# url-kaist/patchwork-plusplus

Hardware: NVIDIA H100
Metric: frames/sec (120k-pt KITTI cloud) (higher is better)
Workload: dtype f64

## Files before the change

### patchwork-plusplus_b200/csrc/pwpp_capi.cu

```cuda
#include <cuda_runtime.h>

#include <sched.h>

#include <algorithm>
#include <cctype>
#include <chrono>
#include <cstdio>
#include <cstdlib>
#include <cstring>
#include <string>
#include <vector>

#include "pwpp.h"
#include "pwpp_kernels.cuh"
#include "pwpp_tuning.h"
#include "pwpp_host.hpp"

using namespace pwpp;

static_assert(sizeof(BinFit) == sizeof(pwpp_bin_result), "BinFit must mirror pwpp_bin_result");

namespace {

thread_local std::string g_last_error;
// ... 509 lines not shown
  pwpp_ctx* ctx = new pwpp_ctx();
  ctx->prm = *params;
  ctx->device = device;
  ctx->num_streams = num_streams;
  build_geometry(*params, ctx->g, ctx->ap, ctx->fast_bin);
  ctx->sw_serial_fit = env_int("PWPP_SERIAL_FIT", 0, 0, 1) != 0;
  ctx->sw_front = env_int("PWPP_FRONT", PWPP_FRONT_DEFAULT, 0, 1);
  ctx->sw_patch = env_int("PWPP_FIT_PATCH", PWPP_FIT_PATCH_DEFAULT, 0, 1);
  ctx->sw_graph = env_int("PWPP_GRAPH", 1, 0, 1);
  ctx->small_call_frames = env_int("PWPP_SMALL_CALL", PWPP_SMALL_CALL_DEFAULT, 0, 64);
  ctx->nbp = ((ctx->g.nbins + PW_NUM_PSEUDO + 31) / 32) * 32;
  int max_sectors = 0;
  for (int k = 0; k < 4; ++k) max_sectors = std::max(max_sectors, ctx->g.num_sectors[k]);
  ctx->hcap = std::max(params->max_elevation_storage, params->max_flatness_storage) + 4 * max_sectors + 64;
  ctx->max_sectors = max_sectors;
#define CU_TRY_CTX(expr)                                                                                  \
  do {                                                                                                    \
    cudaError_t _e = (expr);                                                                              \
    if (_e != cudaSuccess) {                                                                              \
      std::string m = std::string(#expr) + ": " + cudaGetErrorString(_e);                                 \
      pwpp_destroy(ctx);                                                                                  \
      return fail(PWPP_ERR_CUDA, m);                                                                      \
    }                                                                                                     \
  } while (0)
  CU_TRY_CTX(cudaSetDevice(device));
  CU_TRY_CTX(cudaStreamCreateWithFlags(&ctx->stream, cudaStreamNonBlocking));
  CU_TRY_CTX(cudaStreamCreateWithFlags(&ctx->stream_h2d, cudaStreamNonBlocking));
  CU_TRY_CTX(cudaStreamCreateWithFlags(&ctx->stream_d2h, cudaStreamNonBlocking));
  CU_TRY_CTX(cudaEventCreate(&ctx->ev0));
  CU_TRY_CTX(cudaEventCreate(&ctx->ev1));
  CU_TRY_CTX(cudaEventCreate(&ctx->ev_begin));
  CU_TRY_CTX(cudaEventCreate(&ctx->ev_end));
  for (int i = 0; i <= PWPP_NUM_STAGES; ++i) CU_TRY_CTX(cudaEventCreate(&ctx->stage_ev[i]));
  for (int i = 0; i < 2; ++i) CU_TRY_CTX(cudaEventCreateWithFlags(&ctx->tab_ev[i], cudaEventDisableTiming));
  CU_TRY_CTX(cudaEventCreateWithFlags(&ctx->ev_fork, cudaEventDisableTiming));
  for (int q = 0; q < NUM_SIDE; ++q) {
    CU_TRY_CTX(cudaStreamCreateWithFlags(&ctx->side[q], cudaStreamNonBlocking));
    CU_TRY_CTX(cudaEventCreateWithFlags(&ctx->ev_fit[q], cudaEventDisableTiming));
    CU_TRY_CTX(cudaEventCreateWithFlags(&ctx->ev_join[q], cudaEventDisableTiming));
  }
  CU_TRY_CTX(ctx->d_states.reserve(num_streams));
  CU_TRY_CTX(ctx->d_states_init.reserve(num_streams));
  {
    std::vector<StreamState> v(num_streams);
    for (auto& st : v) init_state(*params, st);
    CU_TRY_CTX(cudaMemcpy(ctx->d_states_init.p, v.data(), v.size() * sizeof(StreamState), cudaMemcpyHostToDevice));
  }
  CU_TRY_CTX(ctx->d_hist.reserve((size_t) num_streams * 2 * 4 * ctx->hcap));
  CU_TRY_CTX(ctx->d_counts.reserve((size_t) 3 * num_streams));
  CU_TRY_CTX(ctx->d_wq_ctr.reserve(2 * NUM_CLASSES + ORD_NUM_HEADS));
  {
    cudaDeviceProp prop;
    CU_TRY_CTX(cudaGetDeviceProperties(&prop, device));
    const size_t sm_m = FITW_WARPS * CLS_M_MAX * sizeof(float4), sm_l2 = 3 * 4096 * sizeof(float), sm_l3 = 3 * 8192 * sizeof(float);
    ctx->fit[0] = {k_fit_resident<8, 8, 0, 2>, 0, FIT_THREADS, 0};
    ctx->fit[1] = {k_fit_warp<true, 1, 1, 2, 3, false, true>, 0, FITW_WARPS * 32, sm_m};
    ctx->fit[2] = {k_fit_warp<false, 2, 2, 2, 3, false, true>, 0, FITW_WARPS * 32, 0};
    ctx->fit[3] = {k_fit_cta<4096, 3, 3, 8, true, true>, 0, FIT_THREADS, sm_l2};
    ctx->fit[4] = {k_fit_cta<8192, 4, 2, 8, true>, 0, FIT_THREADS, sm_l3};
    ctx->fit[5] = {k_fit_big<16, 1, true>, 0, 512, 0};
    if (ctx->sw_patch) {
      ctx->fit[2] = {k_fit_patch<4, 4, 2>, 0, 4 * 32, (size_t) 4 * FP_STG * sizeof(float4)};
      ctx->fit[3] = {k_fit_patch<8, 2, 3>, 0, 8 * 32, (size_t) 8 * FP_STG * sizeof(float4)};
      ctx->fit[4] = {k_fit_patch<16, 1, 4>, 0, 16 * 32, (size_t) 16 * FP_STG * sizeof(float4)};
    }
    for (int c = 0; c < NUM_CLASSES; ++c) ctx->fit_small[c] = ctx->fit[c];
    ctx->fit_small[2] = {k_fit_patch<4, 4, 2>, 0, 4 * 32, (size_t) 4 * FP_STG * sizeof(float4)};
    ctx->fit_small[3] = {k_fit_patch<8, 2, 3>, 0, 8 * 32, (size_t) 8 * FP_STG * sizeof(float4)};
    ctx->fit_small[4] = {k_fit_patch<16, 1, 4>, 0, 16 * 32, (size_t) 16 * FP_STG * sizeof(float4)};
    for (int c = 0; c < 2 * NUM_CLASSES; ++c) {
      FitLaunch& k = c < NUM_CLASSES ? ctx->fit[c] : ctx->fit_small[c - NUM_CLASSES];
      if (k.smem > 0) CU_TRY_CTX(cudaFuncSetAttribute(k.fn, cudaFuncAttributeMaxDynamicSharedMemorySize, (int) k.smem));
      int per_sm = 1;
      CU_TRY_CTX(cudaOccupancyMaxActiveBlocksPerMultiprocessor(&per_sm, k.fn, k.threads, k.smem));
      k.grid = std::max(1, per_sm) * prop.multiProcessorCount;
    }
    {
      typedef void (*OrdKernel)(const float4*, WorkQueues, int*, int*);
      const OrdKernel fn[ORD_NUM_HEADS] = {k_order_cta<512, 5>, k_order_cta<512, 4>, k_order_cta<256, 3>, k_order_cta<128, 2>, k_order_warp};
      const int th[ORD_NUM_HEADS] = {512, 512, 256, 128, ORD_WARP_THREADS};
      for (int q = 0; q < ORD_NUM_HEADS; ++q) {
        const size_t sm = q < 4 ? ord_cta_smem_bytes(th[q]) : 0;
        if (sm > 48 * 1024) CU_TRY_CTX(cudaFuncSetAttribute(fn[q], cudaFuncAttributeMaxDynamicSharedMemorySize, (int) sm));
        int per_sm = 1;
        CU_TRY_CTX(cudaOccupancyMaxActiveBlocksPerMultiprocessor(&per_sm, fn[q], th[q], sm));
        ctx->order_k[q].grid = std::max(1, per_sm) * prop.multiProcessorCount;
        ctx->order_k[q].threads = th[q];
        ctx->order_k[q].smem = sm;
      }
    }
    const size_t gle_smem = gle_smem_bytes(max_sectors);
    if (gle_smem > 48 * 1024) CU_TRY_CTX(cudaFuncSetAttribute(k_gle, cudaFuncAttributeMaxDynamicSharedMemorySize, (int) gle_smem));
  }
  {
    const size_t scat = (size_t) (CHUNK_THREADS / 32) * ctx->nbp * sizeof(unsigned int);
    if (scat > 48 * 1024) CU_TRY_CTX(cudaFuncSetAttribute(k_scatter<false, 4>, cudaFuncAttributeMaxDynamicSharedMemorySize, (int) scat));
    const size_t sm_f = front_cluster_smem_bytes(ctx->nbp, FC_THREADS), sm_fd = front_cluster_smem_bytes(ctx->nbp, FC_THREADS_DENSE);
    if (sm_f > 220 * 1024) ctx->sw_front = 0;
    ctx->front_dense_ok = sm_fd <= 220 * 1024;
    if (ctx->sw_front) {
      CU_TRY_CTX(cudaFuncSetAttribute(k_front_cluster<true, CLS_L2_MAX, FC_THREADS>, cudaFuncAttributeMaxDynamicSharedMemorySize, (int) sm_f));
      CU_TRY_CTX(cudaFuncSetAttribute(k_front_cluster<false, CLS_L2_MAX, FC_THREADS>, cudaFuncAttributeMaxDynamicSharedMemorySize, (int) sm_f));
      if (ctx->front_dense_ok) {
        CU_TRY_CTX(cudaFuncSetAttribute(k_front_cluster<true, CLS_L2_MAX, FC_THREADS_DENSE>, cudaFuncAttributeMaxDynamicSharedMemorySize, (int) sm_fd));
        CU_TRY_CTX(cudaFuncSetAttribute(k_front_cluster<false, CLS_L2_MAX, FC_THREADS_DENSE>, cudaFuncAttributeMaxDynamicSharedMemorySize, (int) sm_fd));
      }
    }
// ... 432 lines not shown
  int node = -1;
  if (FILE* f = std::fopen((base + "/numa_node").c_str(), "r")) { if (std::fscanf(f, "%d", &node) != 1) node = -1; std::fclose(f); }
  if (node < 0) return -1;
  std::string list;
  if (FILE* f = std::fopen(("/sys/devices/system/node/node" + std::to_string(node) + "/cpulist").c_str(), "r")) {
    char buf[4096] = {0};
    if (std::fgets(buf, sizeof buf, f)) list = buf;
    std::fclose(f);
  }
  if (list.empty()) return -1;
  cpu_set_t set;
  CPU_ZERO(&set);
  int ncpu = 0;
  const char* p = list.c_str();
  while (*p) {
    char* end = nullptr;
    long a = std::strtol(p, &end, 10);
    if (end == p) break;
    long b = a;
    if (*end == '-') { p = end + 1; b = std::strtol(p, &end, 10); }
    for (long c = a; c <= b && c < CPU_SETSIZE; ++c) { CPU_SET((int) c, &set); ++ncpu; }
    p = (*end == ',') ? end + 1 : end;
    if (*end != ',' ) break;
  }
  if (ncpu == 0 || sched_setaffinity(0, sizeof set, &set) != 0) return -1;
  return node;
}

int pwpp_copy_bin_results(pwpp_ctx* ctx, int f, pwpp_bin_result* dst) {
  int rc = check_frame(ctx, f);
  if (rc) return rc;
  rc = bind_device(ctx);
  if (rc) return rc;
  CU_TRY(cudaStreamSynchronize(ctx->last_stream));
  CU_TRY(cudaMemcpy(dst, ctx->d_fits.p + (size_t) f * ctx->g.nbins, (size_t) ctx->g.nbins * sizeof(BinFit), cudaMemcpyDeviceToHost));
  return PWPP_OK;
}
int pwpp_copy_bin_ids(pwpp_ctx* ctx, int f, uint16_t* dst) {
  int rc = check_frame(ctx, f);
  if (rc) return rc;
  rc = bind_device(ctx);
  if (rc) return rc;
  CU_TRY(cudaStreamSynchronize(ctx->last_stream));
  const int n = frame_n(ctx, f);
  if (n > 0) CU_TRY(cudaMemcpy(dst, ctx->d_bin_ids.p + ctx->pt_off[f], (size_t) n * sizeof(uint16_t), cudaMemcpyDeviceToHost));
  return PWPP_OK;
}

#if defined(PWPP_PHASE_CLOCKS)
int pwpp_debug_phase_clocks(pwpp_ctx* ctx, unsigned long long* out, int reset) {
  if (!ctx) return PWPP_ERR_INVALID_ARG;
  cudaSetDevice(ctx->device);
  cudaDeviceSynchronize();
  if (out) cudaMemcpyFromSymbol(out, g_phase_clk, sizeof(unsigned long long) * 48);
  if (reset) { static unsigned long long z[48]; cudaMemcpyToSymbol(g_phase_clk, z, sizeof z); }
  return PWPP_OK;
}
int pwpp_debug_events(pwpp_ctx* ctx, unsigned* out, int max_events) {
  if (!ctx) return -1;
  cudaSetDevice(ctx->device);
  cudaDeviceSynchronize();
  if (out && max_events >= 16384) cudaMemcpyFromSymbol(out, g_ev, (size_t) 16384 * 16);
  static uint4 z[16384];
  cudaMemcpyToSymbol(g_ev, z, sizeof z);
  return 16384;
}
#endif

}
```

### patchwork-plusplus_b200/csrc/pwpp_common.cuh

```cuda
#pragma once
#include <cuda_runtime.h>

#include "pwpp_gle.cuh"
#include "pwpp_math.cuh"

namespace pwpp {

constexpr int CHUNK_PTS = 4096;
constexpr int CHUNK_THREADS = 256;
constexpr int WARP_PTS = CHUNK_PTS / (CHUNK_THREADS / 32);
constexpr int WARP_ITERS = WARP_PTS / 32;
constexpr int MAX_LPR = 64;
constexpr int MAX_RVPF = 8;

struct FrameTable {
  const long long* pt_off;
  const int* chunk_off;
};

__device__ __forceinline__ int lane_id() { return threadIdx.x & 31; }
#if defined(PWPP_SIMT_EMU)
__device__ __forceinline__ unsigned pw_cluster_rank() { return blockIdx.x; }
__device__ __forceinline__ void pw_cluster_sync() { simt::cluster_sync_(); }
template <typename T> __device__ __forceinline__ T* pw_cluster_map(T* p, unsigned rank) { return static_cast<T*>(simt::cluster_map_(p, (int) rank)); }
#else
}
#include <cooperative_groups.h>
namespace pwpp {
__device__ __forceinline__ unsigned pw_cluster_rank() { return cooperative_groups::this_cluster().block_rank(); }
__device__ __forceinline__ void pw_cluster_sync() { cooperative_groups::this_cluster().sync(); }
template <typename T> __device__ __forceinline__ T* pw_cluster_map(T* p, unsigned rank) { return cooperative_groups::this_cluster().map_shared_rank(p, rank); }
#endif

#if defined(PWPP_SIMT_EMU)
__device__ __forceinline__ unsigned lanemask_lt() { return (1u << (threadIdx.x & 31)) - 1u; }
__device__ __forceinline__ float4 ld_stream_f4(const float4* p) { return *p; }
__device__ __forceinline__ void prefetch_l2(const void*) {}
#else
#define PW_DYN_SHARED(T, name) extern __shared__ T name[]
__device__ __forceinline__ unsigned lanemask_lt() { unsigned m; asm("mov.u32 %0, %%lanemask_lt;" : "=r"(m)); return m; }

__device__ __forceinline__ float4 ld_stream_f4(const float4* p) {
  float4 v;
  asm("ld.global.nc.L1::no_allocate.v4.f32 {%0,%1,%2,%3}, [%4];" : "=f"(v.x), "=f"(v.y), "=f"(v.z), "=f"(v.w) : "l"(p));
  return v;
}
__device__ __forceinline__ void prefetch_l2(const void* p) { asm volatile("prefetch.global.L2 [%0];" ::"l"(p)); }
#endif

#if !defined(PWPP_SIMT_EMU)
__device__ __forceinline__ unsigned smem_u32(const void* p) { return (unsigned) __cvta_generic_to_shared(p); }
__device__ __forceinline__ void mbar_init(unsigned long long* bar, int count) {
  asm volatile("mbarrier.init.shared::cta.b64 [%0], %1;" ::"r"(smem_u32(bar)), "r"(count) : "memory");
}
__device__ __forceinline__ void mbar_expect_tx(unsigned long long* bar, unsigned bytes) {
  asm volatile("mbarrier.arrive.expect_tx.shared::cta.b64 _, [%0], %1;" ::"r"(smem_u32(bar)), "r"(bytes) : "memory");
}
__device__ __forceinline__ void mbar_wait(unsigned long long* bar, unsigned parity) {
  asm volatile(
      "{\n"
      ".reg .pred p;\n"
      "WAIT_%=:\n"
      "mbarrier.try_wait.parity.shared::cta.b64 p, [%0], %1;\n"
      "@p bra DONE_%=;\n"
      "bra WAIT_%=;\n"
      "DONE_%=:\n"
      "}\n" ::"r"(smem_u32(bar)), "r"(parity) : "memory");
}
__device__ __forceinline__ void bulk_g2s(void* dst_smem, const void* src_gmem, unsigned bytes, unsigned long long* bar) {
  asm volatile("cp.async.bulk.shared::cta.global.mbarrier::complete_tx::bytes [%0], [%1], %2, [%3];" ::"r"(smem_u32(dst_smem)), "l"(src_gmem), "r"(bytes),
               "r"(smem_u32(bar))
               : "memory");
}
__device__ __forceinline__ void fence_proxy_async() { asm volatile("fence.proxy.async.shared::cta;" ::: "memory"); }
#endif


}
```

### patchwork-plusplus_b200/csrc/pwpp_fit.cuh

```cuda
#pragma once
#include <cuda_runtime.h>

#include "pwpp_common.cuh"

namespace pwpp {

constexpr int FIT_THREADS = 256;
constexpr int CLS_S_MAX = 64, CLS_M_MAX = 512, CLS_L1_MAX = 2048, CLS_L2_MAX = 4096, CLS_L3_MAX = 8192;
constexpr int NUM_CLASSES = 6;

struct WorkQueues {
  int4* items[NUM_CLASSES];
  int* count;
  int* head;
  unsigned char* labels;
};
#define PW_LABEL_GROUND 255
#define PW_LABEL_REJECT 0
__device__ __forceinline__ int4 make_work_item(int frame, int bin, int n, long long start) {
  return make_int4((frame << 12) | bin, n, (int) (unsigned) (start & 0xffffffffll), (int) (start >> 32));
}
__device__ __forceinline__ long long work_item_start(const int4& w) { return ((long long) w.w << 32) | (long long) (unsigned) w.z; }
__device__ __forceinline__ void prefetch_patch_l2(const float4* P, int n, int lane, int nlanes) {
  const int lines = (n + 7) >> 3;
  for (int l = lane; l < lines; l += nlanes) prefetch_l2(P + (size_t) l * 8);
}

__device__ __forceinline__ unsigned order_key(float z) {
  const unsigned u = __float_as_uint(z);
  return (u & 0x80000000u) ? ~u : (u | 0x80000000u);
}
__device__ __forceinline__ float key_to_float(unsigned k) {
  const unsigned u = (k & 0x80000000u) ? (k & 0x7fffffffu) : ~k;
  return __uint_as_float(u);
}

template <typename F>
__device__ __forceinline__ unsigned kth_key(unsigned kmin, unsigned kmax, int target, F count_less) {
  const unsigned diff = kmin ^ kmax;
  if (diff == 0u) return kmin;
  const int top = 31 - __clz(diff);
  unsigned ans = (top == 31) ? 0u : (kmin & ~((2u << top) - 1u));
  for (int bit = top; bit >= 0; --bit) {
    const unsigned cand = ans | (1u << bit);
    if (count_less(cand) < target) ans = cand;
  }
  return ans;
}

template <int G>
struct GroupOps;

template <>
struct GroupOps<8> {
  __device__ static __forceinline__ unsigned min_u(unsigned v) {
    v = min(v, __shfl_xor_sync(0xffffffffu, v, 4)); v = min(v, __shfl_xor_sync(0xffffffffu, v, 2)); v = min(v, __shfl_xor_sync(0xffffffffu, v, 1));
// ... 759 lines not shown
    for (int j = k >> 1; j > 0; j >>= 1) {
#pragma unroll
      for (int t = 0; t < 2; ++t) {
        const int idx = lane + 32 * t;
        const int i = ((idx & ~(j - 1)) << 1) | (idx & (j - 1));
        const int l = i | j;
        const bool up = ((i & k) == 0);
        const float a = buf[i], b = buf[l];
        if ((a > b) == up) { buf[i] = b; buf[l] = a; }
      }
      __syncwarp();
    }
  }
}

struct LprSelector {
  float* buf;
  int m;
  float tau;
  int K;
  __device__ __forceinline__ void init(float* b, int k) { buf = b; m = 0; tau = INFINITY; K = k; }
  __device__ __forceinline__ void prune() {
    const int lane = lane_id();
    for (int i = m + lane; i < 128; i += 32) buf[i] = INFINITY;
    __syncwarp();
    warp_sort128(buf);
    if (m > K) m = K;
    if (m == K) tau = buf[K - 1];
    __syncwarp();
  }
  __device__ __forceinline__ void push(bool valid, float key) {
    const bool c = valid && (key < tau);
    const unsigned bal = __ballot_sync(0xffffffffu, c);
    if (bal == 0) return;
    if (c) buf[m + __popc(bal & lanemask_lt())] = key;
    m += __popc(bal);
    __syncwarp();
    if (m > 96) prune();
  }
};

struct RvpfPlanes {
  Plane pl[MAX_RVPF];
  int n;
};

__device__ __forceinline__ bool is_alive(const RvpfPlanes& rv, double th_dist_v, float x, float y, float z) {
  bool alive = true;
  for (int k = 0; k < rv.n; ++k) alive = alive && !(fabs(point_plane_distance(rv.pl[k], x, y, z)) < th_dist_v);
  return alive;
}

constexpr int WARP_CAP = CLS_L3_MAX;
constexpr int FITW_WARPS = 8;
constexpr int FITW_U = 4;

__device__ __noinline__ double warp_lpr_fallback(const float4* __restrict__ P, int n, int nit, bool any_removed, const unsigned* __restrict__ alive_w,
                                                 float margin_f, int num_lpr, float* sel_buf) {
  const int lane = lane_id();
  double lpr = 0.0;
  LprSelector sel;
  sel.init(sel_buf, num_lpr);
  for (int it = 0; it < nit; ++it) {
    const int j = it * 32 + lane;
    bool valid = j < n;
    const float z = P[j < n ? j : n - 1].z;
    if (any_removed) valid = valid && ((alive_w[it] >> lane) & 1u);
    if (z < margin_f) valid = false;
    sel.push(valid, z);
  }
  sel.prune();
  if (lane == 0) {
    double sum = 0.0;
    for (int i = 0; i < sel.m; ++i) sum += (double) sel_buf[i];
    lpr = sel.m != 0 ? sum / sel.m : 0.0;
  }
  __syncwarp();
  return __shfl_sync(0xffffffffu, lpr, 0);
}

__device__ double warp_lpr(const float4* __restrict__ P, int n, int nit, bool any_removed, const unsigned* __restrict__ alive_w, float margin_f,
                           int num_lpr, float* sel_buf) {
  const int lane = lane_id();
  const unsigned lt = lanemask_lt();
  unsigned* cbuf = reinterpret_cast<unsigned*>(sel_buf);
  bool fallback = num_lpr > 32;
  double lpr = 0.0;
  if (!fallback) {
    constexpr int LPR_U = 2;
    unsigned kminL = 0xffffffffu;
    int nv = 0;
    for (int it0 = 0; it0 < nit; it0 += LPR_U) {
      float zb[LPR_U];
#pragma unroll
      for (int u = 0; u < LPR_U; ++u) { const int j = (it0 + u) * 32 + lane; zb[u] = P[j < n ? j : n - 1].z; }
#pragma unroll
      for (int u = 0; u < LPR_U; ++u) {
        const int it = it0 + u, j = it * 32 + lane;
        bool valid = j < n;
        const float z = zb[u];
        if (any_removed && it < nit) valid = valid && ((alive_w[it] >> lane) & 1u);
        if (z < margin_f) valid = false;
        if (valid) { kminL = min(kminL, order_key(z)); ++nv; }
      }
    }
    const int nvalid = __reduce_add_sync(0xffffffffu, nv);
    const int target = nvalid < num_lpr ? nvalid : num_lpr;
// ... 6 lines not shown
      T = kth_key(gmn, gmx, target, [&](unsigned cand) { return __reduce_add_sync(0xffffffffu, kminL < cand ? 1 : 0); });
    }
    int cc = 0;
    for (int it0 = 0; it0 < nit; it0 += LPR_U) {
      float zb[LPR_U];
#pragma unroll
      for (int u = 0; u < LPR_U; ++u) { const int j = (it0 + u) * 32 + lane; zb[u] = P[j < n ? j : n - 1].z; }
#pragma unroll
      for (int u = 0; u < LPR_U; ++u) {
        const int it = it0 + u, j = it * 32 + lane;
        bool valid = j < n;
        const float z = zb[u];
        if (any_removed && it < nit) valid = valid && ((alive_w[it] >> lane) & 1u);
        if (z < margin_f) valid = false;
        const unsigned key = order_key(z);
        const bool c = valid && key <= T;
        const unsigned bal = __ballot_sync(0xffffffffu, c);
        if (c) { const int pos = cc + __popc(bal & lt); if (pos < 128) cbuf[pos] = key; }
        cc += __popc(bal);
      }
    }
    __syncwarp();
    if (cc <= 128) {
      unsigned ck[4];
      unsigned kmn = 0xffffffffu, kmx = 0u;
#pragma unroll
      for (int q = 0; q < 4; ++q) {
        const int i = lane + 32 * q;
        ck[q] = i < cc ? cbuf[i] : 0xffffffffu;
        if (i < cc) { kmn = min(kmn, ck[q]); kmx = max(kmx, ck[q]); }
      }
      kmn = __reduce_min_sync(0xffffffffu, kmn);
      kmx = __reduce_max_sync(0xffffffffu, kmx);
      const unsigned ans = kth_key(kmn, kmx, target, [&](unsigned cand) {
        int cnt = 0;
#pragma unroll
        for (int q = 0; q < 4; ++q) cnt += ck[q] < cand;
        return __reduce_add_sync(0xffffffffu, cnt);
      });
      double ps = 0.0;
      int c_lt = 0;
#pragma unroll
      for (int q = 0; q < 4; ++q) if (ck[q] < ans) { ps += (double) key_to_float(ck[q]); ++c_lt; }
      ps = warp_sum(ps);
      c_lt = __reduce_add_sync(0xffffffffu, c_lt);
      lpr = (ps + (double) (target - c_lt) * (double) key_to_float(ans)) / (double) target;
      __syncwarp();
    } else fallback = true;
  }
  if (fallback) lpr = warp_lpr_fallback(P, n, nit, any_removed, alive_w, margin_f, num_lpr, sel_buf);
  return lpr;
}

template <bool STAGE, int CLS_HI, int CLS_LO, int U, int MINB, bool FUSE = false, bool PLS = false>
__global__ void __launch_bounds__(FITW_WARPS * 32, MINB) k_fit_warp(const float4* __restrict__ sorted, FrameTable ft, const StreamState* __restrict__ states,
                                                                             Geometry g, AlgoParams ap, int nbp, const int* __restrict__ bin_off, WorkQueues wq,
                                                                             int* __restrict__ part, BinFit* __restrict__ fits) {
  constexpr int CAP = STAGE ? CLS_M_MAX : (CLS_HI == 2 ? CLS_L1_MAX : WARP_CAP);
  __shared__ unsigned s_alive[FITW_WARPS][CAP / 32];
  __shared__ unsigned s_member[FITW_WARPS][CAP / 32];
  __shared__ float s_sel[FITW_WARPS][128];
  __shared__ Plane s_pl[PLS ? FITW_WARPS : 1];
  __shared__ Moments s_tot[PLS ? FITW_WARPS : 1];
  static_assert(!(PLS && FUSE), "the fused seed round keeps two planes in registers");
  PW_DYN_SHARED(float4, s_stage);
  const int warp = threadIdx.x >> 5, lane = lane_id();
  const unsigned lt = lanemask_lt();
  unsigned* alive_w = s_alive[warp];
  unsigned* member_w = s_member[warp];
  float* sel_buf = s_sel[warp];
  int cls = CLS_HI;
  const int cls_last = CLS_LO;
  const float thf = (float) ap.th_dist;
  int cnt = wq.count[cls];
  const int4 no_item = make_int4(-1, 0, 0, 0);
  int4 cur = no_item;
  auto claim_sync = [&]() {
    cur = no_item;
    while (cls >= cls_last) {
      int t = 0;
      if (lane == 0) t = atomicAdd(&wq.head[cls], 1);
      t = __shfl_sync(0xffffffffu, t, 0);
      if (t < cnt) { cur = wq.items[cls][t]; return; }
      --cls;
      if (cls >= cls_last) cnt = wq.count[cls];
    }
  };
  claim_sync();

  for (;;) {
    if (cur.x < 0) return;
    int next_raw = 0;
    if (lane == 0) next_raw = atomicAdd(&wq.head[cls], 1);
    int4 nxt = no_item;
    bool looked_ahead = false;
    const int f = cur.x >> 12, bin = cur.x & 0xfff, n = cur.y;
    const long long start = work_item_start(cur);
    const float4* G = sorted + start;
    int* out = part + start;
    const int nit = (n + 31) >> 5;
    const float4* P = G;
    if (STAGE) {
      float4* mine = s_stage + warp * CLS_M_MAX;
      for (int it = 0; it < nit; it += FITW_U) {
        float4 q[FITW_U];
#pragma unroll
        for (int u = 0; u < FITW_U; ++u) { const int j = (it + u) * 32 + lane; q[u] = G[j < n ? j : n - 1]; }
#pragma unroll
        for (int u = 0; u < FITW_U; ++u) { const int j = (it + u) * 32 + lane; if (j < n) mine[j] = q[u]; }
      }
      __syncwarp();
      P = mine;
    }
    const int zone = (bin >= g.bin_base[3]) ? 3 : (bin >= g.bin_base[2]) ? 2 : (bin >= g.bin_base[1]) ? 1 : 0;
    const bool zone0 = (zone == 0);
    const float margin_f = zone0 ? float_ru(ap.adaptive_seed_selection_margin * states[f].sensor_height) : -INFINITY;
    const float4 first = P[0];
    double c[3] = {(double) first.x, (double) first.y, 0.0};

    bool have_plane = false, any_removed = false;
    Plane pl_reg;
    Plane& pl = PLS ? s_pl[warp] : pl_reg;
    auto set_plane = [&](const Plane& t) { if (!PLS) pl_reg = t; else { __syncwarp(); if (lane == 0) s_pl[warp] = t; __syncwarp(); } };
    {
      Plane z;
      z.d = 0.0;
#pragma unroll
      for (int q = 0; q < 3; ++q) { z.mean[q] = 0.0; z.normal[q] = 0.0; z.sv[q] = 0.0; }
      set_plane(z);
    }

    Moments tot_reg;
    Moments& tot = PLS ? s_tot[warp] : tot_reg;
    auto set_tot = [&](const Moments& t) { if (!PLS) tot_reg = t; else { __syncwarp(); if (lane == 0) s_tot[warp] = t; __syncwarp(); } };
    int rvpf_left = (ap.enable_RVPF && zone0) ? ap.num_iter : 0;
    const bool fuse_ok = FUSE && (ap.th_seeds <= ap.th_seeds_v);
    for (;;) {
      const bool rvpf_round = rvpf_left > 0;
      const bool fused = fuse_ok && rvpf_round;
      const double lpr = warp_lpr(P, n, nit, any_removed, alive_w, margin_f, ap.num_lpr, sel_buf);
      const float zthr = float_ru(lpr + (rvpf_round ? ap.th_seeds_v : ap.th_seeds));
      const float zin = float_ru(lpr + ap.th_seeds);
      c[2] = lpr;
      if (!looked_ahead) {
        const int t_next = __shfl_sync(0xffffffffu, next_raw, 0);
        if (t_next < cnt) nxt = wq.items[cls][t_next];
        looked_ahead = true;
      }
      Moments m, mi;
      m.n = 0; mi.n = 0;
#pragma unroll
      for (int q = 0; q < 3; ++q) { m.s1[q] = 0.0; mi.s1[q] = 0.0; }
#pragma unroll
      for (int q = 0; q < 6; ++q) { m.s2[q] = 0.0; mi.s2[q] = 0.0; }
      for (int it = 0; it < nit; it += U) {
        float4 q[U];
#pragma unroll
        for (int u = 0; u < U; ++u) { const int j = (it + u) * 32 + lane; q[u] = P[j < n ? j : n - 1]; }
#pragma unroll
        for (int u = 0; u < U; ++u) {
          const int j = (it + u) * 32 + lane;
          const float4 p = q[u];
          bool in = (j < n) && (p.z < zthr);
          if (any_removed && it + u < nit) in = in && ((alive_w[it + u] >> lane) & 1u);
          const unsigned bal = __ballot_sync(0xffffffffu, in);
          unsigned bal_in = bal;
          bool inner = in;
          if (FUSE && fused) { inner = in && (p.z < zin); bal_in = __ballot_sync(0xffffffffu, inner); }
          if (lane == 0 && it + u < nit) member_w[it + u] = bal_in;
          if (bal) {
            const double w = in ? 1.0 : 0.0;
            const double dx = ((double) p.x - c[0]) * w, dy = ((double) p.y - c[1]) * w, dz = ((double) p.z - c[2]) * w;
            m.s1[0] += dx; m.s1[1] += dy; m.s1[2] += dz;
            m.s2[0] += dx * dx; m.s2[1] += dx * dy; m.s2[2] += dx * dz;
            m.s2[3] += dy * dy; m.s2[4] += dy * dz; m.s2[5] += dz * dz;
            m.n += in ? 1 : 0;
            if (FUSE && fused && bal_in) {
              const double wi = inner ? 1.0 : 0.0;
              const double ex = dx * wi, ey = dy * wi, ez = dz * wi;
              mi.s1[0] += ex; mi.s1[1] += ey; mi.s1[2] += ez;
              mi.s2[0] += ex * ex; mi.s2[1] += ex * ey; mi.s2[2] += ex * ez;
              mi.s2[3] += ey * ey; mi.s2[4] += ey * ez; mi.s2[5] += ez * ez;
              mi.n += inner ? 1 : 0;
            }
          }
        }
      }
      group_sum_moments<32>(m, lane);
      m.n = warp_sum_i(m.n);
      if (FUSE && fused) {
        group_sum_moments<32>(mi, lane);
        mi.n = warp_sum_i(mi.n);
        const bool hi = lane >= 16;
        Moments ms;
        ms.n = hi ? mi.n : m.n;
#pragma unroll
        for (int q = 0; q < 3; ++q) ms.s1[q] = hi ? mi.s1[q] : m.s1[q];
#pragma unroll
        for (int q = 0; q < 6; ++q) ms.s2[q] = hi ? mi.s2[q] : m.s2[q];
        Plane mine = pl;
        if (ms.n > 0) plane_from_moments(ms, c, mine);
        auto bcast = [&](int src) {
          Plane t;
#pragma unroll
          for (int q = 0; q < 3; ++q) { t.mean[q] = __shfl_sync(0xffffffffu, mine.mean[q], src); t.normal[q] = __shfl_sync(0xffffffffu, mine.normal[q], src); t.sv[q] = __shfl_sync(0xffffffffu, mine.sv[q], src); }
          t.d = __shfl_sync(0xffffffffu, mine.d, src);
          return t;
        };
        if (m.n > 0) { pl = bcast(0); have_plane = true; }
        if (!(have_plane && pl.normal[2] < ap.uprightness_thr)) {
          if (mi.n > 0) { pl = bcast(16); have_plane = true; }
          set_tot(mi);
          break;
        }
      } else {
        if (m.n > 0) { Plane t; plane_from_moments(m, c, t); set_plane(t); have_plane = true; }
        set_tot(m);
        if (!rvpf_round) break;
      }
      if (have_plane && pl.normal[2] < ap.uprightness_thr) {
        for (int it = 0; it < nit; ++it) {
          const int j = it * 32 + lane;
          bool keep = j < n;
          const float4 p = P[j < n ? j : n - 1];
          if (any_removed) keep = keep && ((alive_w[it] >> lane) & 1u);
          const bool was_alive = keep;
          keep = keep && !(fabs(point_plane_distance(pl, p.x, p.y, p.z)) < ap.th_dist_v);
          if (wq.labels && was_alive && !keep) wq.labels[start + j] = (unsigned char) (ap.num_iter - rvpf_left + 1);
          const unsigned bal = __ballot_sync(0xffffffffu, keep);
          if (lane == 0) alive_w[it] = bal;
        }
        __syncwarp();
        any_removed = true;
        --rvpf_left;
      } else rvpf_left = 0;
    }
    __syncwarp();

    if (nxt.x >= 0) prefetch_patch_l2(sorted + work_item_start(nxt), nxt.y, lane, 32);
    for (int round = 0; round < ap.num_iter && have_plane; ++round) {
      PlaneF pf;
      pf.n0 = (float) pl.normal[0]; pf.n1 = (float) pl.normal[1]; pf.n2 = (float) pl.normal[2]; pf.d = (float) pl.d;
      Moments dm;
      dm.n = 0;
#pragma unroll
      for (int q = 0; q < 3; ++q) dm.s1[q] = 0.0;
#pragma unroll
      for (int q = 0; q < 6; ++q) dm.s2[q] = 0.0;
      unsigned changed_any = 0;
      for (int it = 0; it < nit; it += U) {
        float4 q[U];
#pragma unroll
        for (int u = 0; u < U; ++u) { const int j = (it + u) * 32 + lane; q[u] = P[j < n ? j : n - 1]; }
#pragma unroll
        for (int u = 0; u < U; ++u) {
          if (it + u >= nit) break;
          const int j = (it + u) * 32 + lane;
          const float4 p = q[u];
          int fl = dist_filter(pf, thf, p.x, p.y, p.z);
          if (fl < 0) fl = (point_plane_distance(pl, p.x, p.y, p.z) < ap.th_dist) ? 1 : 0;
          bool in = (j < n) && (fl != 0);
          if (any_removed) in = in && ((alive_w[it + u] >> lane) & 1u);
          const unsigned bal = __ballot_sync(0xffffffffu, in);
          const unsigned prev = member_w[it + u];
          const unsigned chg = bal ^ prev;
          if (chg) {
            changed_any |= chg;
            const bool mine = (chg >> lane) & 1u;
            const double w = mine ? (in ? 1.0 : -1.0) : 0.0;
            const double dx = (double) p.x - c[0], dy = (double) p.y - c[1], dz = (double) p.z - c[2];
            const double wx = dx * w, wy = dy * w, wz = dz * w;
            dm.s1[0] += wx; dm.s1[1] += wy; dm.s1[2] += wz;
            dm.s2[0] += wx * dx; dm.s2[1] += wx * dy; dm.s2[2] += wx * dz;
            dm.s2[3] += wy * dy; dm.s2[4] += wy * dz; dm.s2[5] += wz * dz;
            dm.n += mine ? (in ? 1 : -1) : 0;
            __syncwarp();
            if (lane == 0) member_w[it + u] = bal;
          }
        }
      }
      if (changed_any == 0) break;
      {
        group_sum_moments<32>(dm, lane);
        Moments t = tot;
#pragma unroll
        for (int q = 0; q < 3; ++q) t.s1[q] += dm.s1[q];
#pragma unroll
        for (int q = 0; q < 6; ++q) t.s2[q] += dm.s2[q];
        t.n += warp_sum_i(dm.n);
        set_tot(t);
        if (t.n > 0) { Plane np; plane_from_moments(t, c, np); set_plane(np); }
      }
      __syncwarp();
    }
    const int n_ground = have_plane ? tot.n : 0;
    __syncwarp();
    {
      int g_run = 0, ng_run = 0;
      for (int it0 = 0; it0 < nit; it0 += U) {
        int idxb[U];
#pragma unroll
        for (int u = 0; u < U; ++u) { const int j = (it0 + u) * 32 + lane; idxb[u] = __float_as_int(P[j < n ? j : n - 1].w); }
#pragma unroll
        for (int u = 0; u < U; ++u) {
          const int it = it0 + u, j = it * 32 + lane;
          if (it >= nit) break;
          const bool v = j < n;
          const unsigned bg = have_plane ? member_w[it] : 0u;
          const unsigned bv = __ballot_sync(0xffffffffu, v);
          const unsigned bn = bv & ~bg;
          if (v) {
            const int idx = idxb[u];
            if ((bg >> lane) & 1u) out[g_run + __popc(bg & lt)] = idx;
            else out[n_ground + ng_run + __popc(bn & lt)] = idx;
            if (wq.labels) { const bool isg = (bg >> lane) & 1u; if (isg || !any_removed || ((alive_w[it] >> lane) & 1u)) wq.labels[start + j] = isg ? PW_LABEL_GROUND : PW_LABEL_REJECT; }
          }
          g_run += __popc(bg);
          ng_run += __popc(bn);
        }
      }
    }
    if (lane == 0) {
      BinFit& r = fits[(size_t) f * g.nbins + bin];
      r.n = n; r.n_ground = n_ground; r.fitted = 1;
      r.verdict = have_plane ? 0 : PW_FIT_NO_PLANE;
#pragma unroll
      for (int q = 0; q < 3; ++q) { r.mean[q] = pl.mean[q]; r.normal[q] = pl.normal[q]; r.sv[q] = pl.sv[q]; }
      r.d = pl.d;
    }
    __syncwarp();
    if (nxt.x >= 0) cur = nxt;
    else {
      --cls;
      if (cls >= cls_last) cnt = wq.count[cls];
      claim_sync();
    }
  }
}

}
```

### patchwork-plusplus_b200/csrc/pwpp_trace.cuh

```cuda
#pragma once
#include <cuda_runtime.h>

namespace pwpp {
#if defined(PWPP_PHASE_CLOCKS) && !defined(PWPP_SIMT_EMU)
__device__ unsigned long long g_phase_clk[8][16];
#define PW_CLK_DECL long long _clk_t = clock64(); unsigned long long _clk_acc[12] = {0, 0, 0, 0, 0, 0, 0, 0, 0, 0, 0, 0}
#define PW_CLK(ph) do { if (threadIdx.x == 0) { const long long _n = clock64(); _clk_acc[ph] += (unsigned long long) (_n - _clk_t); _clk_t = _n; } } while (0)
#define PW_CNT(ph) do { if (threadIdx.x == 0) _clk_acc[ph] += 1; } while (0)
#define PW_CLK_FLUSH(cls) do { if (threadIdx.x == 0) for (int _q = 0; _q < 12; ++_q) atomicAdd(&g_phase_clk[cls][_q], _clk_acc[_q]); } while (0)
#ifndef PWPP_TRACE_CLS
#define PWPP_TRACE_CLS 1
#endif
__device__ unsigned g_evn;
__device__ uint4 g_ev[16384];
#define PW_EV_DECL unsigned _evi = 0
#define PW_EV(id) do { if (CLS == PWPP_TRACE_CLS && blockIdx.x == 0 && (threadIdx.x & 31) == 0 && _evi < 1024u) { g_ev[((threadIdx.x >> 5) << 10) + _evi] = make_uint4((unsigned) (id), threadIdx.x >> 5, (unsigned) clock64(), 1u); ++_evi; } } while (0)
#else
#define PW_CLK_DECL
#define PW_CLK(ph)
#define PW_CNT(ph)
#define PW_CLK_FLUSH(cls)
#define PW_EV(id)
#define PW_EV_DECL
#endif
}
```

Measured before the change: 142,800.

## Offload per-warp plane solves to a dedicated solver warp via mbarriers

Adds a ninth warp to the warp-fit kernel that acts as a shared plane solver. Worker warps post their moments and centroid through shared memory and mbarriers, then wait for the solver warp to run plane_from_moments and write back the plane. The fused seed-round path is removed, and phase-clock instrumentation is extended to per-warp slots. The aim is to take the serial double-precision eigen solve off the worker warps and batch it across lanes. The cost is an extra warp per block, handshake latency on every solve, and a polling loop.

```diff
diff --git a/patchwork-plusplus_b200/csrc/pwpp_capi.cu b/patchwork-plusplus_b200/csrc/pwpp_capi.cu
--- a/patchwork-plusplus_b200/csrc/pwpp_capi.cu
+++ b/patchwork-plusplus_b200/csrc/pwpp_capi.cu
@@ -585,7 +585,7 @@
   {
     cudaDeviceProp prop;
     CU_TRY_CTX(cudaGetDeviceProperties(&prop, device));
-    const size_t sm_m = FITW_WARPS * CLS_M_MAX * sizeof(float4), sm_l2 = 3 * 4096 * sizeof(float), sm_l3 = 3 * 8192 * sizeof(float);
+    const size_t sm_m = FITW_PASS * CLS_M_MAX * sizeof(float4), sm_l2 = 3 * 4096 * sizeof(float), sm_l3 = 3 * 8192 * sizeof(float);
     ctx->fit[0] = {k_fit_resident<8, 8, 0, 2>, 0, FIT_THREADS, 0};
     ctx->fit[1] = {k_fit_warp<true, 1, 1, 2, 3, false, true>, 0, FITW_WARPS * 32, sm_m};
     ctx->fit[2] = {k_fit_warp<false, 2, 2, 2, 3, false, true>, 0, FITW_WARPS * 32, 0};
@@ -1124,8 +1124,8 @@
   if (!ctx) return PWPP_ERR_INVALID_ARG;
   cudaSetDevice(ctx->device);
   cudaDeviceSynchronize();
-  if (out) cudaMemcpyFromSymbol(out, g_phase_clk, sizeof(unsigned long long) * 48);
-  if (reset) { static unsigned long long z[48]; cudaMemcpyToSymbol(g_phase_clk, z, sizeof z); }
+  if (out) cudaMemcpyFromSymbol(out, g_phase_clk, sizeof(unsigned long long) * 128);
+  if (reset) { static unsigned long long z[128]; cudaMemcpyToSymbol(g_phase_clk, z, sizeof z); }
   return PWPP_OK;
 }
 int pwpp_debug_events(pwpp_ctx* ctx, unsigned* out, int max_events) {
diff --git a/patchwork-plusplus_b200/csrc/pwpp_common.cuh b/patchwork-plusplus_b200/csrc/pwpp_common.cuh
--- a/patchwork-plusplus_b200/csrc/pwpp_common.cuh
+++ b/patchwork-plusplus_b200/csrc/pwpp_common.cuh
@@ -75,5 +75,38 @@
 __device__ __forceinline__ void fence_proxy_async() { asm volatile("fence.proxy.async.shared::cta;" ::: "memory"); }
 #endif
 
+#if defined(PWPP_SIMT_EMU)
+__device__ __forceinline__ void mbar_init(unsigned long long* bar, int count) { *bar = ((unsigned long long) count << 33) | (unsigned) count; }
+__device__ __forceinline__ void mbar_arrive(unsigned long long* bar) {
+  ++g_cta.progress;
+  const unsigned long long v = *bar, cnt = v >> 33;
+  unsigned long long ph = (v >> 32) & 1u, pend = (v & 0xffffffffull) - 1;
+  if (pend == 0) { ph ^= 1u; pend = cnt; }
+  *bar = (cnt << 33) | (ph << 32) | pend;
+}
+__device__ __forceinline__ bool mbar_test_wait(unsigned long long* bar, unsigned parity) { return ((*bar >> 32) & 1u) != parity; }
+__device__ __forceinline__ void mbar_wait(unsigned long long* bar, unsigned parity) { while (!mbar_test_wait(bar, parity)) simt::yield_(); }
+__device__ __forceinline__ int pw_load_volatile(const int* p) { return *p; }
+__device__ __forceinline__ void pw_backoff() { simt::yield_(); }
+__device__ __forceinline__ void pw_fence_block() {}
+#else
+__device__ __forceinline__ void mbar_arrive(unsigned long long* bar) {
+  asm volatile("mbarrier.arrive.shared::cta.b64 _, [%0];" ::"r"(smem_u32(bar)) : "memory");
+}
+__device__ __forceinline__ bool mbar_test_wait(unsigned long long* bar, unsigned parity) {
+  unsigned r;
+  asm volatile(
+      "{\n"
+      ".reg .pred p;\n"
+      "mbarrier.test_wait.parity.shared::cta.b64 p, [%1], %2;\n"
+      "selp.u32 %0, 1, 0, p;\n"
+      "}\n" : "=r"(r) : "r"(smem_u32(bar)), "r"(parity) : "memory");
+  return r != 0;
+}
+__device__ __forceinline__ int pw_load_volatile(const int* p) { return *(const volatile int*) p; }
+__device__ __forceinline__ void pw_backoff() { __nanosleep(32); }
+__device__ __forceinline__ void pw_fence_block() { __threadfence_block(); }
+#endif
+
 
 }
diff --git a/patchwork-plusplus_b200/csrc/pwpp_fit.cuh b/patchwork-plusplus_b200/csrc/pwpp_fit.cuh
--- a/patchwork-plusplus_b200/csrc/pwpp_fit.cuh
+++ b/patchwork-plusplus_b200/csrc/pwpp_fit.cuh
@@ -2,6 +2,7 @@
 #include <cuda_runtime.h>
 
 #include "pwpp_common.cuh"
+#include "pwpp_trace.cuh"
 
 namespace pwpp {
 
@@ -867,7 +868,6 @@
 }
 
 constexpr int WARP_CAP = CLS_L3_MAX;
-constexpr int FITW_WARPS = 8;
 constexpr int FITW_U = 4;
 
 __device__ __noinline__ double warp_lpr_fallback(const float4* __restrict__ P, int n, int nit, bool any_removed, const unsigned* __restrict__ alive_w,
@@ -980,23 +980,86 @@
   return lpr;
 }
 
-template <bool STAGE, int CLS_HI, int CLS_LO, int U, int MINB, bool FUSE = false, bool PLS = false>
+constexpr int FITW_WARPS = 9;
+constexpr int FITW_PASS = FITW_WARPS - 1;
+template <bool STAGE, int CLS_HI, int CLS_LO, int U, int MINB, bool FUSE = false, bool PLS = true>
 __global__ void __launch_bounds__(FITW_WARPS * 32, MINB) k_fit_warp(const float4* __restrict__ sorted, FrameTable ft, const StreamState* __restrict__ states,
-                                                                             Geometry g, AlgoParams ap, int nbp, const int* __restrict__ bin_off, WorkQueues wq,
-                                                                             int* __restrict__ part, BinFit* __restrict__ fits) {
+                                                                      Geometry g, AlgoParams ap, int nbp, const int* __restrict__ bin_off, WorkQueues wq,
+                                                                      int* __restrict__ part, BinFit* __restrict__ fits) {
+  static_assert(!FUSE && PLS, "the solver warp reads and answers through the shared-memory plane and sums; no fused round");
   constexpr int CAP = STAGE ? CLS_M_MAX : (CLS_HI == 2 ? CLS_L1_MAX : WARP_CAP);
-  __shared__ unsigned s_alive[FITW_WARPS][CAP / 32];
-  __shared__ unsigned s_member[FITW_WARPS][CAP / 32];
-  __shared__ float s_sel[FITW_WARPS][128];
-  __shared__ Plane s_pl[PLS ? FITW_WARPS : 1];
-  __shared__ Moments s_tot[PLS ? FITW_WARPS : 1];
-  static_assert(!(PLS && FUSE), "the fused seed round keeps two planes in registers");
+  __shared__ unsigned s_alive[FITW_PASS][CAP / 32];
+  __shared__ unsigned s_member[FITW_PASS][CAP / 32];
+  __shared__ float s_sel[FITW_PASS][128];
+  __shared__ Plane s_pl[FITW_PASS];
+  __shared__ Moments s_tot[FITW_PASS];
+  __shared__ double s_c[FITW_PASS][3];
+  __shared__ __align__(8) unsigned long long s_req[FITW_PASS], s_ans[FITW_PASS];
+  __shared__ int s_posted;
   PW_DYN_SHARED(float4, s_stage);
   const int warp = threadIdx.x >> 5, lane = lane_id();
+  PW_CLK_DECL;
+  if (warp == FITW_PASS) {
+    if (lane < FITW_PASS) { mbar_init(&s_req[lane], 1); mbar_init(&s_ans[lane], 1); }
+    if (lane == 0) s_posted = 0;
+  }
+  __syncthreads();
+
+  if (warp == FITW_PASS) {
+    bool live = lane < FITW_PASS;
+    unsigned req_ph = 0;
+    for (;;) {
+      const int seen = __shfl_sync(0xffffffffu, pw_load_volatile(&s_posted), 0);
+      const bool pend = live && mbar_test_wait(&s_req[lane], req_ph);
+      if (pend) {
+        req_ph ^= 1u;
+        const Moments m = s_tot[lane];
+        if (m.n == 0) live = false;
+        else {
+          const double c[3] = {s_c[lane][0], s_c[lane][1], s_c[lane][2]};
+          Plane t;
+          plane_from_moments(m, c, t);
+          s_pl[lane] = t;
+          mbar_arrive(&s_ans[lane]);
+        }
+      }
+#if defined(PWPP_PHASE_CLOCKS)
+      {
+        const unsigned solved = __ballot_sync(0xffffffffu, pend && live);
+        PW_CNT(PH_N_BATCHED, __popc(solved));
+        PW_CNT(PH_N_BATCH, solved != 0u ? 1 : 0);
+      }
+#endif
+      if (!__any_sync(0xffffffffu, live)) break;
+      if (__any_sync(0xffffffffu, pend)) { PW_CLK(PH_SOLVER_BUSY); continue; }
+      PW_CLK(PH_SOLVER_BUSY);
+      while (pw_load_volatile(&s_posted) == seen) pw_backoff();
+      PW_CLK(PH_SOLVER_IDLE);
+    }
+    PW_CLK(PH_SOLVER_BUSY);
+    PW_CLK_FLUSH(CLS_HI);
+    return;
+  }
+
   const unsigned lt = lanemask_lt();
   unsigned* alive_w = s_alive[warp];
   unsigned* member_w = s_member[warp];
   float* sel_buf = s_sel[warp];
+  Plane& pl = s_pl[warp];
+  Moments& tot = s_tot[warp];
+  unsigned ans_ph = 0;
+  auto post = [&]() {
+    if (lane == 0) { mbar_arrive(&s_req[warp]); pw_fence_block(); atomicAdd(&s_posted, 1); }
+  };
+  auto set_plane = [&](const Plane& t) { __syncwarp(); if (lane == 0) s_pl[warp] = t; __syncwarp(); };
+  auto set_tot = [&](const Moments& t) { __syncwarp(); if (lane == 0) s_tot[warp] = t; __syncwarp(); };
+  auto solve = [&](const double (&c)[3]) {
+    if (lane == 0) { s_c[warp][0] = c[0]; s_c[warp][1] = c[1]; s_c[warp][2] = c[2]; }
+    post();
+    mbar_wait(&s_ans[warp], ans_ph);
+    ans_ph ^= 1u;
+    PW_CNT(PH_N_SOLVE, 1);
+  };
   int cls = CLS_HI;
   const int cls_last = CLS_LO;
   const float thf = (float) ap.th_dist;
@@ -1017,7 +1080,12 @@
   claim_sync();
 
   for (;;) {
-    if (cur.x < 0) return;
+    if (cur.x < 0) {
+      if (lane == 0) tot.n = 0;
+      post();
+      PW_CLK_FLUSH(CLS_HI);
+      return;
+    }
     int next_raw = 0;
     if (lane == 0) next_raw = atomicAdd(&wq.head[cls], 1);
     int4 nxt = no_item;
@@ -1047,9 +1115,6 @@
     double c[3] = {(double) first.x, (double) first.y, 0.0};
 
     bool have_plane = false, any_removed = false;
-    Plane pl_reg;
-    Plane& pl = PLS ? s_pl[warp] : pl_reg;
-    auto set_plane = [&](const Plane& t) { if (!PLS) pl_reg = t; else { __syncwarp(); if (lane == 0) s_pl[warp] = t; __syncwarp(); } };
     {
       Plane z;
       z.d = 0.0;
@@ -1058,29 +1123,26 @@
       set_plane(z);
     }
 
-    Moments tot_reg;
-    Moments& tot = PLS ? s_tot[warp] : tot_reg;
-    auto set_tot = [&](const Moments& t) { if (!PLS) tot_reg = t; else { __syncwarp(); if (lane == 0) s_tot[warp] = t; __syncwarp(); } };
     int rvpf_left = (ap.enable_RVPF && zone0) ? ap.num_iter : 0;
-    const bool fuse_ok = FUSE && (ap.th_seeds <= ap.th_seeds_v);
+    PW_CLK(PH_STAGE);
+    PW_CNT(PH_N_PATCH, 1);
     for (;;) {
       const bool rvpf_round = rvpf_left > 0;
-      const bool fused = fuse_ok && rvpf_round;
       const double lpr = warp_lpr(P, n, nit, any_removed, alive_w, margin_f, ap.num_lpr, sel_buf);
+      PW_CLK(PH_LPR);
       const float zthr = float_ru(lpr + (rvpf_round ? ap.th_seeds_v : ap.th_seeds));
-      const float zin = float_ru(lpr + ap.th_seeds);
       c[2] = lpr;
       if (!looked_ahead) {
         const int t_next = __shfl_sync(0xffffffffu, next_raw, 0);
         if (t_next < cnt) nxt = wq.items[cls][t_next];
         looked_ahead = true;
       }
-      Moments m, mi;
-      m.n = 0; mi.n = 0;
-#pragma unroll
-      for (int q = 0; q < 3; ++q) { m.s1[q] = 0.0; mi.s1[q] = 0.0; }
-#pragma unroll
-      for (int q = 0; q < 6; ++q) { m.s2[q] = 0.0; mi.s2[q] = 0.0; }
+      Moments m;
+      m.n = 0;
+#pragma unroll
+      for (int q = 0; q < 3; ++q) m.s1[q] = 0.0;
+#pragma unroll
+      for (int q = 0; q < 6; ++q) m.s2[q] = 0.0;
       for (int it = 0; it < nit; it += U) {
         float4 q[U];
 #pragma unroll
@@ -1092,10 +1154,7 @@
           bool in = (j < n) && (p.z < zthr);
           if (any_removed && it + u < nit) in = in && ((alive_w[it + u] >> lane) & 1u);
           const unsigned bal = __ballot_sync(0xffffffffu, in);
-          unsigned bal_in = bal;
-          bool inner = in;
-          if (FUSE && fused) { inner = in && (p.z < zin); bal_in = __ballot_sync(0xffffffffu, inner); }
-          if (lane == 0 && it + u < nit) member_w[it + u] = bal_in;
+          if (lane == 0 && it + u < nit) member_w[it + u] = bal;
           if (bal) {
             const double w = in ? 1.0 : 0.0;
             const double dx = ((double) p.x - c[0]) * w, dy = ((double) p.y - c[1]) * w, dz = ((double) p.z - c[2]) * w;
@@ -1103,49 +1162,17 @@
             m.s2[0] += dx * dx; m.s2[1] += dx * dy; m.s2[2] += dx * dz;
             m.s2[3] += dy * dy; m.s2[4] += dy * dz; m.s2[5] += dz * dz;
             m.n += in ? 1 : 0;
-            if (FUSE && fused && bal_in) {
-              const double wi = inner ? 1.0 : 0.0;
-              const double ex = dx * wi, ey = dy * wi, ez = dz * wi;
-              mi.s1[0] += ex; mi.s1[1] += ey; mi.s1[2] += ez;
-              mi.s2[0] += ex * ex; mi.s2[1] += ex * ey; mi.s2[2] += ex * ez;
-              mi.s2[3] += ey * ey; mi.s2[4] += ey * ez; mi.s2[5] += ez * ez;
-              mi.n += inner ? 1 : 0;
-            }
-          }
-        }
-      }
+          }
+        }
+      }
+      PW_CLK(PH_PASS);
       group_sum_moments<32>(m, lane);
       m.n = warp_sum_i(m.n);
-      if (FUSE && fused) {
-        group_sum_moments<32>(mi, lane);
-        mi.n = warp_sum_i(mi.n);
-        const bool hi = lane >= 16;
-        Moments ms;
-        ms.n = hi ? mi.n : m.n;
-#pragma unroll
-        for (int q = 0; q < 3; ++q) ms.s1[q] = hi ? mi.s1[q] : m.s1[q];
-#pragma unroll
-        for (int q = 0; q < 6; ++q) ms.s2[q] = hi ? mi.s2[q] : m.s2[q];
-        Plane mine = pl;
-        if (ms.n > 0) plane_from_moments(ms, c, mine);
-        auto bcast = [&](int src) {
-          Plane t;
-#pragma unroll
-          for (int q = 0; q < 3; ++q) { t.mean[q] = __shfl_sync(0xffffffffu, mine.mean[q], src); t.normal[q] = __shfl_sync(0xffffffffu, mine.normal[q], src); t.sv[q] = __shfl_sync(0xffffffffu, mine.sv[q], src); }
-          t.d = __shfl_sync(0xffffffffu, mine.d, src);
-          return t;
-        };
-        if (m.n > 0) { pl = bcast(0); have_plane = true; }
-        if (!(have_plane && pl.normal[2] < ap.uprightness_thr)) {
-          if (mi.n > 0) { pl = bcast(16); have_plane = true; }
-          set_tot(mi);
-          break;
-        }
-      } else {
-        if (m.n > 0) { Plane t; plane_from_moments(m, c, t); set_plane(t); have_plane = true; }
-        set_tot(m);
-        if (!rvpf_round) break;
-      }
+      set_tot(m);
+      PW_CLK(PH_REDUCE);
+      if (m.n > 0) { solve(c); have_plane = true; }
+      PW_CLK(PH_SOLVE);
+      if (!rvpf_round) break;
       if (have_plane && pl.normal[2] < ap.uprightness_thr) {
         for (int it = 0; it < nit; ++it) {
           const int j = it * 32 + lane;
@@ -1159,6 +1186,7 @@
           if (lane == 0) alive_w[it] = bal;
         }
         __syncwarp();
+        PW_CLK(PH_PASS);
         any_removed = true;
         --rvpf_left;
       } else rvpf_left = 0;
@@ -1207,6 +1235,7 @@
           }
         }
       }
+      PW_CLK(PH_PASS);
       if (changed_any == 0) break;
       {
         group_sum_moments<32>(dm, lane);
@@ -1217,7 +1246,9 @@
         for (int q = 0; q < 6; ++q) t.s2[q] += dm.s2[q];
         t.n += warp_sum_i(dm.n);
         set_tot(t);
-        if (t.n > 0) { Plane np; plane_from_moments(t, c, np); set_plane(np); }
+        PW_CLK(PH_REDUCE);
+        if (t.n > 0) solve(c);
+        PW_CLK(PH_SOLVE);
       }
       __syncwarp();
     }
@@ -1257,6 +1288,7 @@
       r.d = pl.d;
     }
     __syncwarp();
+    PW_CLK(PH_PART);
     if (nxt.x >= 0) cur = nxt;
     else {
       --cls;
diff --git a/patchwork-plusplus_b200/csrc/pwpp_trace.cuh b/patchwork-plusplus_b200/csrc/pwpp_trace.cuh
--- a/patchwork-plusplus_b200/csrc/pwpp_trace.cuh
+++ b/patchwork-plusplus_b200/csrc/pwpp_trace.cuh
@@ -2,12 +2,26 @@
 #include <cuda_runtime.h>
 
 namespace pwpp {
+enum PhaseSlot {
+  PH_STAGE = 0,
+  PH_LPR = 1,
+  PH_PASS = 2,
+  PH_REDUCE = 3,
+  PH_SOLVE = 4,
+  PH_PART = 5,
+  PH_SOLVER_BUSY = 6,
+  PH_SOLVER_IDLE = 7,
+  PH_N_PATCH = 8,
+  PH_N_SOLVE = 9,
+  PH_N_BATCH = 10,
+  PH_N_BATCHED = 11
+};
 #if defined(PWPP_PHASE_CLOCKS) && !defined(PWPP_SIMT_EMU)
 __device__ unsigned long long g_phase_clk[8][16];
 #define PW_CLK_DECL long long _clk_t = clock64(); unsigned long long _clk_acc[12] = {0, 0, 0, 0, 0, 0, 0, 0, 0, 0, 0, 0}
-#define PW_CLK(ph) do { if (threadIdx.x == 0) { const long long _n = clock64(); _clk_acc[ph] += (unsigned long long) (_n - _clk_t); _clk_t = _n; } } while (0)
-#define PW_CNT(ph) do { if (threadIdx.x == 0) _clk_acc[ph] += 1; } while (0)
-#define PW_CLK_FLUSH(cls) do { if (threadIdx.x == 0) for (int _q = 0; _q < 12; ++_q) atomicAdd(&g_phase_clk[cls][_q], _clk_acc[_q]); } while (0)
+#define PW_CLK(ph) do { if ((threadIdx.x & 31) == 0) { const long long _n = clock64(); _clk_acc[ph] += (unsigned long long) (_n - _clk_t); _clk_t = _n; } } while (0)
+#define PW_CNT(ph, v) do { if ((threadIdx.x & 31) == 0) _clk_acc[ph] += (unsigned long long) (v); } while (0)
+#define PW_CLK_FLUSH(cls) do { if ((threadIdx.x & 31) == 0) for (int _q = 0; _q < 12; ++_q) atomicAdd(&g_phase_clk[cls][_q], _clk_acc[_q]); } while (0)
 #ifndef PWPP_TRACE_CLS
 #define PWPP_TRACE_CLS 1
 #endif
@@ -18,7 +32,7 @@
 #else
 #define PW_CLK_DECL
 #define PW_CLK(ph)
-#define PW_CNT(ph)
+#define PW_CNT(ph, v)
 #define PW_CLK_FLUSH(cls)
 #define PW_EV(id)
 #define PW_EV_DECL
```

Result: no change. 143,300 (median of 6 runs) (+0.4%).
